# fengranMark/HAConvDR

Hardware: AMD Instinct MI355X
Metric: queries/sec (encode+top-100) over N-passage 768-d corpus; HBM GB/s vs peak (higher is better)
Workload: dtype bf16 MFMA operands with fp32 accumulate / LayerNorm / softmax in the encoder (cosine vs the fp32 reference within 1e-3, measured ~1e-5); search scores and order = the fp32 fmaf chain, bit-exact

## Files before the change

haconvdr_amd/csrc/gemm8.inc:

```

enum { EPI8_QKV = 0, EPI8_RESID = 2, EPI8_GELU = 3 };
#ifndef G8_N1
#define G8_N1 4
#endif

struct Gemm8Args {
    const bf16 *A;
    const bf16 *W;
    int N, K;
    int n_groups;
    int n_tile0;
    const int *total_rows;
    const float2 *astats;
    const float *wsum;
    const float *cvec;
    bf16 *q, *k, *v16;
    const bf16 *resid;
    const float2 *rstats;
    const float *rgamma, *rbeta;
    bf16 *yb;
    float2 *part;
    bf16 *h;
    unsigned long long *clk;
    int stagger;
    int stagger_mode;
};

__device__ __forceinline__ void glds16(const bf16 *src, unsigned char *dst) {
    typedef const __attribute__((address_space(1))) void *gvp;
    typedef __attribute__((address_space(3))) void *lvp;
    __builtin_amdgcn_global_load_lds((gvp)src, (lvp)dst, 16, 0, 0);
}
__device__ __forceinline__ void swap16(unsigned &a, unsigned &b) {
    const auto r = __builtin_amdgcn_permlane16_swap(a, b, false, false);
    a = r[0];
    b = r[1];
}
__device__ __forceinline__ void quad_transpose4(f4v &v, int p) {
    int x0 = __float_as_int(v.x), x1 = __float_as_int(v.y), x2 = __float_as_int(v.z), x3 = __float_as_int(v.w);
    {
        const bool odd = p & 1;
        const int sa = odd ? x0 : x1, sb = odd ? x2 : x3;
        const int ra = __builtin_amdgcn_update_dpp(0, sa, 0xB1, 0xF, 0xF, false);
        const int rb = __builtin_amdgcn_update_dpp(0, sb, 0xB1, 0xF, 0xF, false);
        x0 = odd ? ra : x0;
        x1 = odd ? x1 : ra;
        x2 = odd ? rb : x2;
        x3 = odd ? x3 : rb;
    }
    {
        const bool hi = p & 2;
        const int sa = hi ? x0 : x2, sb = hi ? x1 : x3;
        const int ra = __builtin_amdgcn_update_dpp(0, sa, 0x4E, 0xF, 0xF, false);
        const int rb = __builtin_amdgcn_update_dpp(0, sb, 0x4E, 0xF, 0xF, false);
        x0 = hi ? ra : x0;
        x2 = hi ? x2 : ra;
        x1 = hi ? rb : x1;
        x3 = hi ? x3 : rb;
    }
    v.x = __int_as_float(x0);
    v.y = __int_as_float(x1);
    v.z = __int_as_float(x2);
    v.w = __int_as_float(x3);
}

__device__ __forceinline__ void xchg8(uint4 &a, uint4 &b, bool lo) {
    unsigned *pa = reinterpret_cast<unsigned *>(&a), *pb = reinterpret_cast<unsigned *>(&b);
#pragma unroll
    for (int i = 0; i < 4; ++i) {
        const unsigned send = lo ? pb[i] : pa[i];
        const unsigned recv = (unsigned)__builtin_amdgcn_update_dpp(0, (int)send, 0x128, 0xF, 0xF, false);
        pa[i] = lo ? pa[i] : recv;
        pb[i] = lo ? recv : pb[i];
    }
}

typedef unsigned g8_u4 __attribute__((ext_vector_type(4)));
typedef unsigned g8_u2 __attribute__((ext_vector_type(2)));
template <bool NT> __device__ __forceinline__ void g8_store16(void *p, uint4 v) {
    if constexpr (NT) __builtin_nontemporal_store(g8_u4{v.x, v.y, v.z, v.w}, reinterpret_cast<g8_u4 *>(p));
    else *reinterpret_cast<uint4 *>(p) = v;
}
template <bool NT> __device__ __forceinline__ void g8_store8(void *p, uint2 v) {
    if constexpr (NT) __builtin_nontemporal_store(g8_u2{v.x, v.y}, reinterpret_cast<g8_u2 *>(p));
    else *reinterpret_cast<uint2 *>(p) = v;
}

__device__ __forceinline__ unsigned pack_bf16(float lo, float hi) {
    typedef __bf16 bf16x2_t __attribute__((ext_vector_type(2)));
    bf16x2_t v;
    v.x = (bf16)lo;
    v.y = (bf16)hi;
    return __builtin_bit_cast(unsigned, v);
}

__device__ __forceinline__ f2v gelu8_2(f2v x) {
    f2v z = x * 0.70710678118654752f;
    z.x = __builtin_amdgcn_fmed3f(z.x, -3.0f, 3.0f);
    z.y = __builtin_amdgcn_fmed3f(z.y, -3.0f, 3.0f);
    const f2v u = z * z;
    f2v p = u * (-1.546677965e-07f) + 6.9032217e-06f;
    p = p * u + (-0.0001336812065f);
    p = p * u + 0.001487465865f;
    p = p * u + (-0.0106578986f);
    p = p * u + 0.0524059485f;
    p = p * u + (-0.1851637965f);
    p = p * u + 0.56346134f;
    return x * (z * p + 0.5f);
}

template <int EPI, bool NT>
__global__ __launch_bounds__(512, 2) void gemm8_kernel(Gemm8Args g) {
    extern __shared__ __attribute__((aligned(16))) unsigned char smem[];
    const int tid = threadIdx.x, lane = tid & 63;
    const int w = __builtin_amdgcn_readfirstlane(tid >> 6);
    const int wr = w >> 2, wc = w & 3;
    if constexpr (EPI == EPI8_GELU) {
        if (g.clk && blockIdx.x == 0 && tid == 0) {
            g.clk[0] = __builtin_amdgcn_s_memtime();
            g.clk[1] = __builtin_amdgcn_s_memrealtime();
        }
    }
    const int K = g.K, KT = K >> 6, nx = (g.N >> 8) - g.n_tile0;
    const int NG = g.n_groups, nxg = nx / NG, NP = 8 / NG;
    const int xcd = blockIdx.x & 7, slot = blockIdx.x >> 3, per_xcd = (gridDim.x + 7 - xcd) >> 3;
    const int mt_all = (*g.total_rows + 255) >> 8;
    const int mt_lo = (int)((long)mt_all * (xcd / NG) / NP), mt_hi = (int)((long)mt_all * (xcd / NG + 1) / NP);
    const int n_base = g.n_tile0 + (xcd % NG) * nxg;
    const int run_lo = 0, run_hi = (mt_hi - mt_lo) * nxg;
    const int tile0 = run_lo + slot;
    if (tile0 >= run_hi) return;
    const int my_tiles = (run_hi - tile0 + per_xcd - 1) / per_xcd;
    const int srow = lane >> 3;
    const int sch0 = (lane & 7) ^ (srow >> 1);
    const int chE = sch0 * 8, chO = (sch0 ^ 4) * 8;
    int s_tile = tile0, s_kt = 0;
    const bf16 *s_A = g.A + (size_t)((mt_lo + s_tile / nxg) << 8) * K, *s_W = g.W + (size_t)((n_base + s_tile % nxg) << 8) * K;
    const int wq = w & 3;
    const unsigned lsrcE = (unsigned)(((wr ? wq * 64 : wq * 32) + srow) * K + chE);
    const unsigned lsrcO = (unsigned)(((wr ? wq * 64 : wq * 32) + 8 + srow) * K + chO);
    const int ring_base = (wr ? 98304 : 0) + wq * 4096, ring_slots = wr ? 4 : 6;
    int h_half = 0, h_slot = 0, h_p = 0;
    const bf16 *h_base = wr ? s_W : s_A;
    long h_left = (long)my_tiles * KT * 8;
    constexpr int N1 = G8_N1, N2 = 8 - N1;
    auto issue_piece = [&]() __attribute__((always_inline)) {
        const bf16 *src = h_base + (size_t)(h_half * (wr ? 32 : 128) + (h_p >> 1) * 16) * K + s_kt * 64;
        unsigned char *dst = smem + ring_base + (h_slot << 14) + h_p * 1024;
        glds16(src + ((h_p & 1) ? lsrcO : lsrcE), dst);
        if (++h_p == 4) {
            h_p = 0;
            h_slot = h_slot + 1 == ring_slots ? 0 : h_slot + 1;
            if (++h_half == 2) {
                h_half = 0;
                if (++s_kt == KT) {
                    s_kt = 0;
                    s_tile += per_xcd;
                    h_base = wr ? g.W + (size_t)((n_base + s_tile % nxg) << 8) * K : g.A + (size_t)((mt_lo + s_tile / nxg) << 8) * K;
                }
            }
        }
    };
    auto issue_pieces = [&](auto ntag) __attribute__((always_inline)) -> bool {
        constexpr int n = decltype(ntag)::value;
        if (h_left <= 0) return false;
        h_left -= n;
#pragma unroll
        for (int i = 0; i < n; ++i) issue_piece();
        return true;
    };
    constexpr std::integral_constant<int, N1> n1tag{};
    constexpr std::integral_constant<int, 16> n16tag{};

    const int m16 = lane & 15, kg = lane >> 4, sw = (m16 >> 1) & 7;
    const int c0 = ((kg ^ sw) << 4), c1 = (((4 + kg) ^ sw) << 4);
    const int a_row = (wr * 64 + m16) * 128, w_row = (wc * 32 + m16) * 128;

#ifdef G8_STAMP
    unsigned long long stamps[16] = {0, 0, 0, 0, 0, 0, 0, 0, 0, 0, 0, 0, 0, 0, 0, 0};
    unsigned long long est[16] = {0, 0, 0, 0, 0, 0, 0, 0, 0, 0, 0, 0, 0, 0, 0, 0};
#define G8_T(i, cond) if (cond) stamps[i] = __builtin_amdgcn_s_memtime()
#define G8_E(i) if (seq == 2) est[i] = __builtin_amdgcn_s_memtime()
#else
#define G8_E(i)
#define G8_T(i, cond)
#endif
#ifdef G8_STAMP2
    unsigned long long ph[16] = {0, 0, 0, 0, 0, 0, 0, 0, 0, 0, 0, 0, 0, 0, 0, 0};
#define G8_P(i) if (seq == 3 && kt == 6) ph[i] = __builtin_amdgcn_s_memtime()
#else
#define G8_P(i)
#endif
    constexpr bool RL = EPI == EPI8_RESID;
    f32x4 acc[2][2][4][2];
    bf16x8 wf0[2][2], wf1[2][2], af0[4][2];

    issue_pieces(n16tag);
    if (g.stagger) {
        const int ph = g.stagger_mode == 0 ? (xcd & 3) : g.stagger_mode == 1 ? (slot & 3) : g.stagger_mode == 2 ? xcd : (slot & 7);
        for (int i = ph * g.stagger; i > 0; --i) __builtin_amdgcn_s_sleep(32);
    }
    asm volatile("s_waitcnt vmcnt(0)" ::: "memory");
    __builtin_amdgcn_s_barrier();

    int a_cur = 0, w_cur = 0;
    for (int seq = 0; seq < my_tiles; ++seq) {
        const int tile = tile0 + seq * per_xcd;
        const int m0 = (mt_lo + tile / nxg) << 8, n0 = (n_base + tile % nxg) << 8;
        unsigned char *R1 = smem, *R2 = smem, *R3 = smem;
        const size_t rl_tb = (size_t)m0 * H + n0;
        auto rl_issue_sb = [&](int i, int mt, unsigned char *dst) __attribute__((always_inline)) {
            int ln = lane;
            asm volatile("" : "+v"(ln));
            const unsigned lo = (unsigned)((ln & 15) * H + (ln >> 5) * 16 + ((ln >> 4) & 1) * 8);
#if defined(G8_RL_ABL) && (G8_RL_ABL & 2)
            const bf16 *src = g.resid + (size_t)(wr * 64 + i * 128 + mt * 16) * H + wc * 64 + lo;
#else
            const bf16 *src = g.resid + (rl_tb + (size_t)(wr * 64 + i * 128 + mt * 16) * H + wc * 64) + lo;
#endif
            glds16(src, dst);
            glds16(src + 32, dst + 1024);
        };
        auto rl_issue_cols = [&](unsigned char *dst) __attribute__((always_inline)) {
            int ln = lane;
            asm volatile("" : "+v"(ln));
            const unsigned so = (unsigned)((ln >> 5) * 128 + 2 * (ln & 31));
            glds16(reinterpret_cast<const bf16 *>(g.rstats + ((size_t)m0 + wr * 64) + so), dst);
            const int sel = (ln >> 4) & 3;
            const float *pc = g.cvec, *pg = g.rgamma, *pb = g.rbeta;
            asm volatile("" : "+s"(pc), "+s"(pg), "+s"(pb));
            const float *vb = pc;
            vb = sel == 1 ? pg : vb;
            vb = sel == 2 ? pb : vb;
            glds16(reinterpret_cast<const bf16 *>(vb + (n0 + wc * 64) + 4 * (ln & 15)), dst + 1024);
        };
        G8_T(2, seq == 3);
        if (wr == 1) __builtin_amdgcn_s_barrier();
#pragma unroll
        for (int i = 0; i < 2; ++i)
#pragma unroll
            for (int j = 0; j < 2; ++j)
#pragma unroll
                for (int mt = 0; mt < 4; ++mt)
#pragma unroll
                    for (int nt = 0; nt < 2; ++nt)
#pragma unroll
                        for (int e = 0; e < 4; ++e) acc[i][j][mt][nt][e] = 0.f;

        for (int kt = 0; kt < KT; ++kt) {
            G8_P(0);
            const unsigned char *kbA = smem + a_cur * 32768, *kbW = smem + 98304 + w_cur * 32768;
            const bool lastk = RL && kt == KT - 1;
            const bool live1 = (wr == 0 || kt) && h_left > 0 && !(lastk && wr == 0);
            if (live1) {
                h_left -= N1;
#pragma unroll
                for (int i = 0; i < N1; ++i) issue_piece();
            }
            if constexpr (RL) {
                if (lastk) {
                    R1 = smem + (a_cur == 0 ? 2 : a_cur - 1) * 32768 + w * 4096;
                    R3 = smem + a_cur * 32768 + w * 4096;
                    R2 = smem + 98304 + w_cur * 32768 + w * 4096;
                    rl_issue_cols(R1);
                    rl_issue_sb(0, 0, R1 + 2048);
                }
            }
            __builtin_amdgcn_sched_barrier(0);
            G8_P(12);
#pragma unroll
            for (int nt = 0; nt < 2; ++nt) {
                wf0[nt][0] = *reinterpret_cast<const bf16x8 *>(kbW + w_row + nt * 2048 + c0);
                wf0[nt][1] = *reinterpret_cast<const bf16x8 *>(kbW + w_row + nt * 2048 + c1);
                wf1[nt][0] = *reinterpret_cast<const bf16x8 *>(kbW + 16384 + w_row + nt * 2048 + c0);
                wf1[nt][1] = *reinterpret_cast<const bf16x8 *>(kbW + 16384 + w_row + nt * 2048 + c1);
            }
#pragma unroll
            for (int mt = 0; mt < 4; ++mt) {
                af0[mt][0] = *reinterpret_cast<const bf16x8 *>(kbA + a_row + mt * 2048 + c0);
                af0[mt][1] = *reinterpret_cast<const bf16x8 *>(kbA + a_row + mt * 2048 + c1);
            }
            __builtin_amdgcn_sched_barrier(0);
            G8_P(1);
            G8_P(2);
            asm volatile("s_waitcnt lgkmcnt(0)" ::: "memory");
            G8_P(3);
            __builtin_amdgcn_s_barrier();
            G8_P(4);
            G8_T(3 + (kt < 3 ? kt : 3), seq == 3 && kt < 4);
            __builtin_amdgcn_sched_barrier(0);
            __builtin_amdgcn_s_setprio(1);
#pragma unroll
            for (int ks = 0; ks < 2; ++ks)
#pragma unroll
                for (int mt = 0; mt < 4; ++mt)
#pragma unroll
                    for (int nt = 0; nt < 2; ++nt) {
                        acc[0][0][mt][nt] = __builtin_amdgcn_mfma_f32_16x16x32_bf16(wf0[nt][ks], af0[mt][ks], acc[0][0][mt][nt], 0, 0, 0);
                        acc[0][1][mt][nt] = __builtin_amdgcn_mfma_f32_16x16x32_bf16(wf1[nt][ks], af0[mt][ks], acc[0][1][mt][nt], 0, 0, 0);
                    }
            __builtin_amdgcn_s_setprio(0);
            G8_P(5);
            __builtin_amdgcn_s_barrier();
            G8_P(6);
            const bool live2 = h_left > 0 && !lastk;
            if (live2) {
                h_left -= N2;
#pragma unroll
                for (int i = 0; i < N2; ++i) issue_piece();
            }
            if constexpr (RL) {
                if (lastk) {
                    rl_issue_sb(0, 1, R2);
                    rl_issue_sb(0, 2, R2 + 2048);
                }
            }
            __builtin_amdgcn_sched_barrier(0);
            G8_P(13);
#pragma unroll
            for (int mt = 0; mt < 4; ++mt) {
                af0[mt][0] = *reinterpret_cast<const bf16x8 *>(kbA + 16384 + a_row + mt * 2048 + c0);
                af0[mt][1] = *reinterpret_cast<const bf16x8 *>(kbA + 16384 + a_row + mt * 2048 + c1);
            }
            __builtin_amdgcn_sched_barrier(0);
            G8_P(7);
            if (lastk) {
            } else if (kt) {
                if (!live2) asm volatile("s_waitcnt vmcnt(0)" ::: "memory");
                else if (wr == 0) asm volatile("s_waitcnt vmcnt(8)" ::: "memory");
                else asm volatile("s_waitcnt vmcnt(%0)" ::"n"(N2) : "memory");
            }
            asm volatile("s_waitcnt lgkmcnt(0)" ::: "memory");
            G8_P(8);
            __builtin_amdgcn_s_barrier();
            G8_P(9);
            __builtin_amdgcn_sched_barrier(0);
            __builtin_amdgcn_s_setprio(1);
#pragma unroll
            for (int ks = 0; ks < 2; ++ks)
#pragma unroll
                for (int mt = 0; mt < 4; ++mt)
#pragma unroll
                    for (int nt = 0; nt < 2; ++nt) {
                        acc[1][0][mt][nt] = __builtin_amdgcn_mfma_f32_16x16x32_bf16(wf0[nt][ks], af0[mt][ks], acc[1][0][mt][nt], 0, 0, 0);
                        acc[1][1][mt][nt] = __builtin_amdgcn_mfma_f32_16x16x32_bf16(wf1[nt][ks], af0[mt][ks], acc[1][1][mt][nt], 0, 0, 0);
                    }
            __builtin_amdgcn_s_setprio(0);
            G8_P(10);
            __builtin_amdgcn_s_barrier();
            G8_P(11);
            a_cur = a_cur == 2 ? 0 : a_cur + 1;
            w_cur ^= 1;
        }
        G8_T(8, seq == 2 && true);
        if (wr == 0) __builtin_amdgcn_s_barrier();
        G8_T(0, seq == 2);
        if constexpr (!RL) {
            if (wr == 1) issue_pieces(n1tag);
            asm volatile("s_waitcnt vmcnt(0)" ::: "memory");
        }
        G8_T(1, seq == 2);

#ifdef G8_NO_EPI
#pragma unroll
        for (int i = 0; i < 2; ++i)
#pragma unroll
            for (int j = 0; j < 2; ++j)
#pragma unroll
                for (int mt = 0; mt < 4; ++mt)
#pragma unroll
                    for (int nt = 0; nt < 2; ++nt) asm volatile("" ::"v"(acc[i][j][mt][nt]));
        continue;
#endif
        {
            const int colg = 8 * ((kg & 1) * 2 + (kg >> 1));
            if constexpr (RL) {
                const bool lo8 = m16 < 8;
                const unsigned lane_b = (unsigned)((wr * 64 + (m16 & 7)) * H + wc * 64 + (m16 >> 3) * 32 + colg);
                const unsigned rd_off = (unsigned)(((kg >> 1) * 16 + m16) * 16);
                const bool rd_hi = kg & 1;
#define G8_VM(n) asm volatile("s_waitcnt vmcnt(" #n ")" ::: "memory")
#define G8_VMC(c, a, b) do { if (c) G8_VM(a); else G8_VM(b); } while (0)
#define G8_LDS_DONE() asm volatile("s_waitcnt lgkmcnt(0)" ::: "memory")
                constexpr std::integral_constant<int, -1> cnone{};
                constexpr std::integral_constant<int, 0> c0t{};
                constexpr std::integral_constant<int, 1> c1t{};
                constexpr std::integral_constant<int, 2> c2t{};
                constexpr std::integral_constant<int, 3> c3t{};
                constexpr std::integral_constant<int, 8> n8tag{};
                rl_issue_sb(0, 3, R3);
                rl_issue_sb(1, 0, R3 + 2048);
                G8_E(0);
                G8_VM(8);
                G8_E(1);
                float mean_[2][4], rstd_[2][4];
                f4v rg[2][2], rb[2][2];
#pragma unroll
                for (int i = 0; i < 2; ++i)
#pragma unroll
                    for (int mt = 0; mt < 4; ++mt) {
                        g8_u4 c = *reinterpret_cast<const g8_u4 *>(R1 + i * 512 + (mt * 16 + (m16 & 14)) * 8);
                        asm volatile("" : "+v"(c));
                        asm volatile("v_mov_b32 %0, %1" : "=v"(mean_[i][mt]) : "v"((m16 & 1) ? c.z : c.x));
                        asm volatile("v_mov_b32 %0, %1" : "=v"(rstd_[i][mt]) : "v"((m16 & 1) ? c.w : c.y));
                    }
#pragma unroll
                for (int jj = 0; jj < 2; ++jj)
#pragma unroll
                    for (int nt = 0; nt < 2; ++nt) {
                        const int co = (jj * 32 + nt * 16 + 4 * kg) * 4;
                        const f4v cvv = *reinterpret_cast<const f4v *>(R1 + 1024 + co);
#pragma unroll
                        for (int i = 0; i < 2; ++i)
#pragma unroll
                            for (int mt = 0; mt < 4; ++mt) acc[i][jj][mt][nt] += cvv;
                        rg[jj][nt] = *reinterpret_cast<const f4v *>(R1 + 1024 + 256 + co);
                        rb[jj][nt] = *reinterpret_cast<const f4v *>(R1 + 1024 + 512 + co);
                    }
                auto sb_read = [&](const unsigned char *sb, g8_u4 (&c)[2][2]) __attribute__((always_inline)) {
#pragma unroll
                    for (int jj = 0; jj < 2; ++jj) {
                        c[jj][0] = *reinterpret_cast<const g8_u4 *>(sb + jj * 1024 + rd_off);
                        c[jj][1] = *reinterpret_cast<const g8_u4 *>(sb + jj * 1024 + 512 + rd_off);
                        asm volatile("" : "+v"(c[jj][0]), "+v"(c[jj][1]));
                    }
                };
                auto sb_do = [&](auto itag, auto mttag, unsigned char *sb, auto refilltag, const g8_u4 (*pre)[2]) __attribute__((always_inline)) {
                    constexpr int i = decltype(itag)::value, mt = decltype(mttag)::value, refill = decltype(refilltag)::value;
                    const float mean = mean_[i][mt], rstd = rstd_[i][mt];
                    uint4 ro[2];
                    float s1 = 0.f, s2 = 0.f;
                    g8_u4 cc[2][2];
                    if (pre) {
#pragma unroll
                        for (int jj = 0; jj < 2; ++jj) cc[jj][0] = pre[jj][0], cc[jj][1] = pre[jj][1];
                    } else {
                        sb_read(sb, cc);
                    }
#pragma unroll
                    for (int jj = 0; jj < 2; ++jj) {
                        const g8_u4 c0 = cc[jj][0], c1 = cc[jj][1];
                        const uint2 w0 = {rd_hi ? c0.z : c0.x, rd_hi ? c0.w : c0.y}, w1 = {rd_hi ? c1.z : c1.x, rd_hi ? c1.w : c1.y};
                        const f4v ra = {__uint_as_float(w0.x << 16), __uint_as_float(w0.x & 0xffff0000u), __uint_as_float(w0.y << 16), __uint_as_float(w0.y & 0xffff0000u)};
                        const f4v rb_ = {__uint_as_float(w1.x << 16), __uint_as_float(w1.x & 0xffff0000u), __uint_as_float(w1.y << 16), __uint_as_float(w1.y & 0xffff0000u)};
                        const f4v o0 = acc[i][jj][mt][0] + ((ra - mean) * rstd * rg[jj][0] + rb[jj][0]);
                        const f4v o1 = acc[i][jj][mt][1] + ((rb_ - mean) * rstd * rg[jj][1] + rb[jj][1]);
                        unsigned p0 = pack_bf16(o0.x, o0.y), p1 = pack_bf16(o0.z, o0.w);
                        unsigned p2 = pack_bf16(o1.x, o1.y), p3 = pack_bf16(o1.z, o1.w);
                        swap16(p0, p2);
                        swap16(p1, p3);
                        ro[jj] = make_uint4(p0, p1, p2, p3);
                        const f4v sm = o0 + o1, sq = o0 * o0 + o1 * o1;
                        const float t1 = (sm.x + sm.y) + (sm.z + sm.w), t2 = (sq.x + sq.y) + (sq.z + sq.w);
                        s1 = jj ? s1 + t1 : t1;
                        s2 = jj ? s2 + t2 : t2;
                    }
                    s1 += __shfl_xor(s1, 16);
                    s2 += __shfl_xor(s2, 16);
                    s1 += __shfl_xor(s1, 32);
                    s2 += __shfl_xor(s2, 32);
                    xchg8(ro[0], ro[1], lo8);
                    G8_LDS_DONE();
                    if constexpr (refill >= 0) rl_issue_sb(1, refill, sb);
                    __builtin_amdgcn_sched_barrier(0);
                    const size_t row = (size_t)m0 + i * 128 + wr * 64 + mt * 16 + m16;
#if defined(G8_RL_ABL) && (G8_RL_ABL & 1)
                    if (lane == 0) g.part[row * (g.N >> 6) + (n0 >> 6) + wc] = make_float2(s1, s2);
#pragma unroll
                    for (int jj = 0; jj < 2; ++jj)
                        if (lane == 0) g8_store16<NT>(g.yb + rl_tb + (size_t)((i * 128 + mt * 16 + jj * 8) * H) + lane_b, ro[jj]);
#else
                    if (kg == 0) g.part[row * (g.N >> 6) + (n0 >> 6) + wc] = make_float2(s1, s2);
#pragma unroll
                    for (int jj = 0; jj < 2; ++jj)
                        g8_store16<NT>(g.yb + rl_tb + (size_t)((i * 128 + mt * 16 + jj * 8) * H) + lane_b, ro[jj]);
#endif
                    __builtin_amdgcn_sched_barrier(0);
                };
                __builtin_amdgcn_sched_barrier(0);
                bool gA = false, gW = false;
                sb_do(c0t, c0t, R1 + 2048, cnone, nullptr);
                G8_E(2);
                __builtin_amdgcn_s_barrier();
                if (wr == 0) gA = issue_pieces(n8tag);
                __builtin_amdgcn_sched_barrier(0);
                G8_E(3);
                G8_VMC(gA, 17, 9);
                G8_E(4);
                sb_do(c0t, c1t, R2, c1t, nullptr);
                G8_VMC(gA, 20, 12);
                G8_E(5);
                sb_do(c0t, c2t, R2 + 2048, c2t, nullptr);
                G8_VMC(gA, 23, 15);
                G8_E(6);
                sb_do(c0t, c3t, R3, c3t, nullptr);
                G8_VMC(gA, 26, 18);
                G8_E(7);
                sb_do(c1t, c0t, R3 + 2048, cnone, nullptr);
                G8_VM(16);
                G8_E(8);
                sb_do(c1t, c1t, R2, cnone, nullptr);
                G8_VM(14);
                G8_E(9);
                sb_do(c1t, c2t, R2 + 2048, cnone, nullptr);
                G8_E(10);
                G8_VM(12);
                G8_E(11);
                g8_u4 c7[2][2];
                sb_read(R3, c7);
                G8_LDS_DONE();
                __builtin_amdgcn_s_barrier();
                if (wr == 1) gW = issue_pieces(n8tag);
                __builtin_amdgcn_sched_barrier(0);
                G8_E(12);
                sb_do(c1t, c3t, R3, cnone, c7);
                G8_E(13);
                G8_VMC(gW, 3, 27);
                G8_E(14);
                G8_E(15);
#undef G8_VM
#undef G8_VMC
#undef G8_LDS_DONE
            } else {
                float2 st[2][4];
#pragma unroll
                for (int i = 0; i < 2; ++i)
#pragma unroll
                    for (int mt = 0; mt < 4; ++mt) st[i][mt] = g.astats[(size_t)m0 + i * 128 + wr * 64 + mt * 16 + m16];
                const int ldo = EPI == EPI8_GELU ? g.N : H;
                const bool lo8 = m16 < 8;
                const unsigned lane_b = (unsigned)((wr * 64 + (m16 & 7)) * ldo + wc * 64 + (m16 >> 3) * 32 + colg);
                f4v ws[2][2], cv[2][2];
#pragma unroll
                for (int j = 0; j < 2; ++j)
#pragma unroll
                    for (int nt = 0; nt < 2; ++nt) {
                        const int nb = n0 + wc * 64 + j * 32;
                        cv[j][nt] = *reinterpret_cast<const f4v *>(g.cvec + nb + nt * 16 + 4 * kg);
                        ws[j][nt] = *reinterpret_cast<const f4v *>(g.wsum + nb + nt * 16 + 4 * kg);
                    }
#pragma unroll
                for (int i = 0; i < 2; ++i)
#pragma unroll
                    for (int mt = 0; mt < 4; ++mt) {
                        const float nm = -st[i][mt].x * st[i][mt].y;
                        float rs = st[i][mt].y;
                        asm volatile("v_mov_b32 %0, %1" : "=v"(rs) : "v"(st[i][mt].y));
                        uint4 o[2];
#pragma unroll
                        for (int j = 0; j < 2; ++j) {
                            const int nb = n0 + wc * 64 + j * 32;
                            unsigned p[4];
#pragma unroll
                            for (int nt = 0; nt < 2; ++nt) {
                                f4v v = acc[i][j][mt][nt] * rs + (ws[j][nt] * nm + cv[j][nt]);
                                if (EPI == EPI8_QKV && n0 >= 2 * H) {
                                    quad_transpose4(v, lane & 3);
                                    const int n = nb + nt * 16 + 4 * kg + (lane & 3) - 2 * H;
                                    const size_t mg = (size_t)(m0 + i * 128 + wr * 64 + mt * 16) >> 4;
                                    uint2 o2;
                                    o2.x = pack_bf16(v.x, v.y);
                                    o2.y = pack_bf16(v.z, v.w);
                                    g8_store8<NT>(g.v16 + (mg * H + n) * 16 + (m16 & 12), o2);
                                    continue;
                                }
                                if constexpr (EPI == EPI8_GELU) {
                                    const f2v g0 = gelu8_2((f2v){v.x, v.y}), g1 = gelu8_2((f2v){v.z, v.w});
                                    p[2 * nt] = pack_bf16(g0.x, g0.y);
                                    p[2 * nt + 1] = pack_bf16(g1.x, g1.y);
                                } else {
                                    p[2 * nt] = pack_bf16(v.x, v.y);
                                    p[2 * nt + 1] = pack_bf16(v.z, v.w);
                                }
                            }
                            if (EPI == EPI8_QKV && n0 >= 2 * H) continue;
                            swap16(p[0], p[2]);
                            swap16(p[1], p[3]);
                            o[j] = make_uint4(p[0], p[1], p[2], p[3]);
                        }
                        if (EPI == EPI8_QKV && n0 >= 2 * H) continue;
                        xchg8(o[0], o[1], lo8);
                        const size_t ur = (size_t)(m0 + i * 128 + mt * 16) * ldo;
#pragma unroll
                        for (int j = 0; j < 2; ++j) {
                            if constexpr (EPI == EPI8_GELU) {
                                g8_store16<NT>(g.h + ur + (size_t)(j * 8) * ldo + n0 + lane_b, o[j]);
                            } else {
                                bf16 *dst = n0 < H ? g.q + ur + n0 : g.k + ur + (n0 - H);
                                g8_store16<NT>(dst + (size_t)(j * 8) * ldo + lane_b, o[j]);
                            }
                        }
                    }
            }
        }
    }
    if constexpr (EPI == EPI8_GELU) {
        if (g.clk && blockIdx.x == 0 && tid == 0) {
            g.clk[2] = __builtin_amdgcn_s_memtime();
            g.clk[3] = __builtin_amdgcn_s_memrealtime();
        }
    }
#ifdef G8_STAMP2
    if (blockIdx.x == 8 && lane == 0 && (w == 0 || w == 4)) {
        unsigned long long *o = reinterpret_cast<unsigned long long *>(g.part) + 64 + (w ? 16 : 0);
        for (int i = 0; i < 16; ++i) o[i] = ph[i];
    }
#endif
#ifdef G8_STAMP
    if (blockIdx.x == 8 && lane == 0 && (w == 0 || w == 4)) {
        unsigned long long *o = reinterpret_cast<unsigned long long *>(g.part) + (w ? 16 : 0);
        for (int i = 0; i < 16; ++i) o[i] = stamps[i];
        for (int i = 0; i < 16; ++i) o[32 + i] = est[i];
    }
#endif
}

__global__ __launch_bounds__(256) void ln_combine_kernel(const float2 *__restrict__ part, int n_part, int n_cols, const int *__restrict__ total_rows,
                                                         float eps, float2 *__restrict__ stats) {
    const size_t row = (size_t)blockIdx.x * 256 + threadIdx.x;
    if (row >= (size_t)((*total_rows + 255) & ~255)) return;
    float s1 = 0.f, s2 = 0.f;
    if ((n_part & 1) == 0) {
        const float4 *p4 = reinterpret_cast<const float4 *>(part + row * n_part);
        float4 v[8];
        const int n4 = n_part >> 1;
#pragma unroll
        for (int i = 0; i < 8; ++i) v[i] = i < n4 ? p4[i] : make_float4(0.f, 0.f, 0.f, 0.f);
#pragma unroll
        for (int i = 0; i < 8; ++i) {
            s1 += v[i].x + v[i].z;
            s2 += v[i].y + v[i].w;
        }
        for (int i = 16; i < n_part; ++i) {
            const float2 p = part[row * n_part + i];
            s1 += p.x;
            s2 += p.y;
        }
    } else {
        for (int i = 0; i < n_part; ++i) {
            const float2 p = part[row * n_part + i];
            s1 += p.x;
            s2 += p.y;
        }
    }
    const float mean = s1 / n_cols;
    const float var = fmaxf(s2 / n_cols - mean * mean, 0.f);
    stats[row] = make_float2(mean, rsqrtf(var + eps));
}

__global__ __launch_bounds__(256) void fold_ln_kernel(const float *__restrict__ Wf, const float *__restrict__ bias, const float *__restrict__ gamma,
                                                      const float *__restrict__ beta, int K, float scale, bf16 *__restrict__ Wb,
                                                      float *__restrict__ wsum, float *__restrict__ cvec) {
    __shared__ float red[2][4];
    const int n = blockIdx.x, tid = threadIdx.x;
    float s = 0.f, c = 0.f;
    for (int k = tid; k < K; k += 256) {
        const float wv = Wf[(size_t)n * K + k];
        const bf16 wb = (bf16)(wv * (gamma ? gamma[k] : 1.f) * scale);
        Wb[(size_t)n * K + k] = wb;
        s += (float)wb;
        if (beta) c += beta[k] * wv;
    }
    s = wave_sum(s);
    c = wave_sum(c);
    if ((tid & 63) == 0) {
        red[0][tid >> 6] = s;
        red[1][tid >> 6] = c;
    }
    __syncthreads();
    if (tid == 0) {
        wsum[n] = gamma ? (red[0][0] + red[0][1]) + (red[0][2] + red[0][3]) : 0.f;
        cvec[n] = (bias[n] + (red[1][0] + red[1][1]) + (red[1][2] + red[1][3])) * scale;
    }
}

__global__ void fill_identity_stats_kernel(float2 *__restrict__ stats, size_t n) {
    const size_t i = (size_t)blockIdx.x * blockDim.x + threadIdx.x;
    if (i < n) stats[i] = make_float2(0.f, 1.f);
}
```

Measured before the change: 8420.

## Stage non-residual epilogue stats and column vectors through LDS and defer next-tile prefetch

For the QKV and GELU epilogues, the per-row LayerNorm stats and the cvec/wsum column vectors are now fetched into a free half of the W buffer by an async global-to-LDS copy on the last k-iteration. They are then read from LDS instead of through scattered global loads in the epilogue. The next tile's W pieces are issued after a barrier inside the epilogue rather than before it, so that load overlaps the epilogue math and stores. This relies on N1 == 4 so the staging slot is not overwritten, and it adds a barrier plus hand-tuned vmcnt waits that must match the outstanding store and load counts.

```diff
diff --git a/haconvdr_amd/csrc/gemm8.inc b/haconvdr_amd/csrc/gemm8.inc
--- a/haconvdr_amd/csrc/gemm8.inc
+++ b/haconvdr_amd/csrc/gemm8.inc
@@ -225,9 +225,9 @@
             int ln = lane;
             asm volatile("" : "+v"(ln));
             const unsigned so = (unsigned)((ln >> 5) * 128 + 2 * (ln & 31));
-            glds16(reinterpret_cast<const bf16 *>(g.rstats + ((size_t)m0 + wr * 64) + so), dst);
+            glds16(reinterpret_cast<const bf16 *>((RL ? g.rstats : g.astats) + ((size_t)m0 + wr * 64) + so), dst);
             const int sel = (ln >> 4) & 3;
-            const float *pc = g.cvec, *pg = g.rgamma, *pb = g.rbeta;
+            const float *pc = g.cvec, *pg = RL ? g.rgamma : g.wsum, *pb = RL ? g.rbeta : g.wsum;
             asm volatile("" : "+s"(pc), "+s"(pg), "+s"(pb));
             const float *vb = pc;
             vb = sel == 1 ? pg : vb;
@@ -247,6 +247,8 @@
 #pragma unroll
                         for (int e = 0; e < 4; ++e) acc[i][j][mt][nt][e] = 0.f;
 
+        int kt_patch = KT - 1;
+        if constexpr (!RL) asm volatile("" : "+s"(kt_patch));
         for (int kt = 0; kt < KT; ++kt) {
             G8_P(0);
             const unsigned char *kbA = smem + a_cur * 32768, *kbW = smem + 98304 + w_cur * 32768;
@@ -331,6 +333,9 @@
                 else asm volatile("s_waitcnt vmcnt(%0)" ::"n"(N2) : "memory");
             }
             asm volatile("s_waitcnt lgkmcnt(0)" ::: "memory");
+            if constexpr (!RL) {
+                if (kt == kt_patch) rl_issue_cols(smem + 98304 + w_cur * 32768 + 16384 + w * 2048);
+            }
             G8_P(8);
             __builtin_amdgcn_s_barrier();
             G8_P(9);
@@ -355,10 +360,7 @@
         G8_T(8, seq == 2 && true);
         if (wr == 0) __builtin_amdgcn_s_barrier();
         G8_T(0, seq == 2);
-        if constexpr (!RL) {
-            if (wr == 1) issue_pieces(n1tag);
-            asm volatile("s_waitcnt vmcnt(0)" ::: "memory");
-        }
+        if constexpr (!RL) asm volatile("s_waitcnt vmcnt(0)" ::: "memory");
         G8_T(1, seq == 2);
 
 #ifdef G8_NO_EPI
@@ -522,11 +524,15 @@
 #undef G8_VMC
 #undef G8_LDS_DONE
             } else {
+                static_assert(N1 == 4, "the patch lives in the half-slot that the N1 pieces behind the k-loop restage: a whole W half");
+                const unsigned char *EP = smem + 98304 + (w_cur ^ 1) * 32768 + 16384 + w * 2048;
                 float2 st[2][4];
 #pragma unroll
                 for (int i = 0; i < 2; ++i)
 #pragma unroll
-                    for (int mt = 0; mt < 4; ++mt) st[i][mt] = g.astats[(size_t)m0 + i * 128 + wr * 64 + mt * 16 + m16];
+                    for (int mt = 0; mt < 4; ++mt) {
+                        st[i][mt] = *reinterpret_cast<const float2 *>(EP + i * 512 + (mt * 16 + m16) * 8);
+                    }
                 const int ldo = EPI == EPI8_GELU ? g.N : H;
                 const bool lo8 = m16 < 8;
                 const unsigned lane_b = (unsigned)((wr * 64 + (m16 & 7)) * ldo + wc * 64 + (m16 >> 3) * 32 + colg);
@@ -535,10 +541,25 @@
                 for (int j = 0; j < 2; ++j)
 #pragma unroll
                     for (int nt = 0; nt < 2; ++nt) {
-                        const int nb = n0 + wc * 64 + j * 32;
-                        cv[j][nt] = *reinterpret_cast<const f4v *>(g.cvec + nb + nt * 16 + 4 * kg);
-                        ws[j][nt] = *reinterpret_cast<const f4v *>(g.wsum + nb + nt * 16 + 4 * kg);
-                    }
+                        const int co = (j * 32 + nt * 16 + 4 * kg) * 4;
+                        cv[j][nt] = *reinterpret_cast<const f4v *>(EP + 1024 + co);
+                        ws[j][nt] = *reinterpret_cast<const f4v *>(EP + 1024 + 256 + co);
+                    }
+                __builtin_amdgcn_sched_barrier(0);
+#pragma unroll
+                for (int i = 0; i < 2; ++i)
+#pragma unroll
+                    for (int mt = 0; mt < 4; ++mt) asm volatile("" : "+v"(st[i][mt].x), "+v"(st[i][mt].y));
+#pragma unroll
+                for (int j = 0; j < 2; ++j)
+#pragma unroll
+                    for (int nt = 0; nt < 2; ++nt) asm volatile("" : "+v"(cv[j][nt]), "+v"(ws[j][nt]));
+                asm volatile("s_waitcnt lgkmcnt(0)" ::: "memory");
+                G8_E(1);
+                __builtin_amdgcn_s_barrier();
+                bool gW = false;
+                if (wr == 1) gW = issue_pieces(n1tag);
+                __builtin_amdgcn_sched_barrier(0);
 #pragma unroll
                 for (int i = 0; i < 2; ++i)
 #pragma unroll
@@ -591,6 +612,12 @@
                             }
                         }
                     }
+                G8_E(2);
+                if (gW) {
+                    if (EPI == EPI8_QKV && n0 >= 2 * H) asm volatile("s_waitcnt vmcnt(32)" ::: "memory");
+                    else asm volatile("s_waitcnt vmcnt(16)" ::: "memory");
+                }
+                G8_E(3);
             }
         }
     }
```

New measurement: 8473, median of 6. About the same (+0.6%).
